# crowsonkb/style-transfer-pytorch

Hardware: AMD Instinct MI355X
Metric: optimizer iterations/sec (higher is better)
Workload: dtype f32 (3x3 convs: fp16x3 split-plane MFMA, fp32 accumulate); 1 GPU; 512x512 single-scale hot loop (closure + Adam + clamp + EMA), 1 style image 512x512, VGG-19 synthetic weights, max pooling; parallelism=single GPU

## Files before the change

include/st_amd.h:

```cpp
#ifndef ST_AMD_H
#define ST_AMD_H

#ifdef __cplusplus
extern "C" {
#endif

#define ST_AMD_ABI_VERSION 2

#define ST_NUM_CONVS 13
#define ST_NUM_STYLE_LAYERS 5
#define ST_CONTENT_LAYER 22
#define ST_NUM_LOSS_TERMS 7

enum st_pooling { ST_POOL_MAX = 0, ST_POOL_AVERAGE = 1, ST_POOL_L2 = 2 };

typedef struct st_net st_net;
typedef struct st_plan st_plan;

const char* st_last_error(void);
int st_abi_version(void);
const char* st_compiled_arch(void);
long long st_max_pixels(void);
int st_has_experiments(void);
int st_env_switches(const char** names, int capacity);
// ... 125 lines not shown
int st_fabric_selftest(st_fabric* fabric, void* stream, int timeout_ms);
int st_plan_closure_run(st_plan* plan, st_fabric* fabric, void* stream);
long long st_qn_strip_state_bytes(long long count, int world);
int st_qn_strip_dots(void* state, long long count, int rank, int world, const float* grad, st_exchange* gather,
                     void* stream);
int st_qn_strip_apply(void* state, long long count, int world, float* image, const float* grad, float* ema_value,
                      double ema_decay, void* stream);
int st_plan_qn_strip_step(st_plan* plan, st_fabric* fabric, float* image, float* grad, void* state, float* ema_value,
                          double ema_decay, void* stream);
int st_plan_losses(st_plan* plan, float** losses);
int st_plan_term_losses(st_plan* plan, float** terms, int* count);
int st_plan_forward_begin(st_plan* plan, const float* image, int last_layer);
int st_plan_moment_sums(st_plan* plan, int layer, float* sums, void* stream);

int st_plan_set_graph(st_plan* plan, int enable);

int st_plan_profile_enable(st_plan* plan, int enable);
int st_plan_profile_read(st_plan* plan, long long* launches, double* millis, double* flops);
int st_plan_profile_read_hbm(st_plan* plan, int category, long long* launches, double* millis, double* bytes);

int st_op_sqrtm_ns(const float* a, float* root, int n, void* stream);
int st_op_sqrtm_ns_backward(const float* root, const float* grad_root, float* grad_a, int n, void* stream);
int st_op_sqrtm_ns_backward_diag(const float* root, float grad_diag, float* grad_a, int n, void* stream);
int st_op_tv_loss(const float* image, int height, int width, float* loss_out, float* grad_out, void* stream);
int st_op_conv3x3(const float* in, const float* weight, const float* bias, float* out, int cin, int cout,
                  int height, int width, int relu, int precision, void* stream);
int st_op_conv3x3_dgrad(const float* grad_out, const float* relu_out, const float* weight, float* grad_in,
                        int cin, int cout, int height, int width, int precision, void* stream);
int st_op_conv3x3_strip(const float* in, const float* halo, int has_up, int has_down, const float* weight,
                        const float* bias, float* out, int cin, int cout, int height, int width, int relu, int dgrad,
                        int precision, void* stream);
int st_op_conv3x3_strip_ex(const float* in, const float* halo, int has_up, int has_down, const float* weight,
                           const float* bias, float* out, const float* out_mask, int cin, int cout, int height, int width,
                           int relu, int dgrad, int accumulate, int overlap, int precision, void* stream);

int st_op_conv1x1(const float* in, const float* weight, const float* bias, float* out, int cin, int cout,
                  long long npix, int precision, void* stream);

int st_op_pool2x2(const float* in, float* out, int channels, int height, int width, int mode, void* stream);
int st_op_pool2x2_backward(const float* in, const float* grad_out, float* grad_in, int channels, int height, int width,
                           int mode, void* stream);


typedef struct st_head st_head;
int st_head_create(st_head** out, int kind, int channels, int height, int width, int precision);
int st_head_destroy(st_head* head);
// ... 96 lines not shown
```

style-transfer-pytorch_amd/csrc/st_common.h:

```cpp
#pragma once

#include <hip/hip_runtime.h>

#include <algorithm>
#include <atomic>
#include <cstdarg>
#include <cstdio>
#include <string>

namespace st {

typedef float f32x16 __attribute__((ext_vector_type(16)));
typedef float f32x4 __attribute__((ext_vector_type(4)));
typedef float f32x2 __attribute__((ext_vector_type(2)));

constexpr int kWave = 64;

void set_error(const char* fmt, ...);
const char* get_error();

#define ST_HIP(expr)                                                                           \
    do {                                                                                       \
        hipError_t _e = (expr);                                                                \
        if (_e != hipSuccess) {                                                                \
// ... 106 lines not shown
    const float *mean, *mean_t, *cov, *cov_t, *root;
    int n;
    float weight;
    float* loss_out;
    float* gdiag_out;
};
__device__ __forceinline__ float w2_gdiag(const W2LossJob& j) { return -2.f * (j.weight / (float)j.n); }
__device__ __forceinline__ void w2_loss_block(const W2LossJob& j, float* scratch) {
#pragma clang fp contract(off)
    float sm = 0.f, sc = 0.f;
    for (int i = threadIdx.x; i < j.n; i += 256) {
        const float d = j.mean[i] - j.mean_t[i];
        sm += d * d;
        const size_t ii = (size_t)i * j.n + i;
        sc += (j.cov_t[ii] + j.cov[ii]) - 2.f * j.root[ii];
    }
    sm = block_sum_256(sm, scratch);
    sc = block_sum_256(sc, scratch);
    if (threadIdx.x == 0) {
        const float fn = (float)j.n;
        j.loss_out[0] = (sm / fn + sc / fn) * j.weight;
        j.gdiag_out[0] = w2_gdiag(j);
    }
}

static inline int ceil_div(int a, int b) { return (a + b - 1) / b; }

struct ConvProblem {
    const float* in;
    const float* mask;
    const float* wgt;
    const float* bias;
    float* out;
    int cin, cout, height, width;
    int taps;
    int relu;
    int accumulate;
    float* scratch;
    const float* in_halo;
    int has_up, has_down;
    int tune;
    const void* wgt_split;
    int planes;
    int elem;
    unsigned int* amax_word;
    int amax_measure;
// ... 129 lines not shown
int launch_pool_bwd(const float* in, const float* grad_out, float* grad_in, int channels, int height,
                    int width, int mode, hipStream_t s);

struct GramWorkspace {
    float* partial;
    float* partial_sum;
    int max_splits;
};
int gram_choose_splits(int channels, long long npix, int max_splits);
long long gram_per_split(long long npix, int splits);
bool gram_wide_tiles(int channels, long long npix);
int launch_gram_partial(const float* feat, int channels, long long npix, int splits, GramWorkspace ws,
                        hipStream_t s, const unsigned int* bound = nullptr, const float* sqrt_mask = nullptr);
int launch_gram_finalize(GramWorkspace ws, int channels, long long npix, int splits, float* mean, float* srm,
                         hipStream_t s, float* cov = nullptr, float cov_eps = 0.f,
                         float mask_sum = 0.f);

enum GemmEpilogue {
    EPI_SCALE = 0,
    EPI_IDENT_MINUS = 1,
    EPI_DIFF = 2,
    EPI_DEV_SQRT_SCALE = 3
};
struct GemmProblem {
    const float* a1; const float* b1;
    const float* a2; const float* b2; const float* b2sub;
    float* d;
    int ta1, tb1, ta2;
    int epilogue;
    float c, ci;
    const float* dev_scalar;
    int n;
    float* sumsq_partials;
};
bool gemm_sumsq_fusable(int n);
struct GemmBatch {
    GemmProblem p[6];
    int count;
    int n;
};
int launch_gemm_batch(const GemmBatch& b, hipStream_t s);
bool head_dgrad_small_applies(int channels, long long npix);
int launch_head_dgrad_small(const float* ssym, const float* feat, const float* bias, const float* mask, float* out, int channels,
                            long long npix, unsigned int* out_amax, hipStream_t s);

struct NSWorkspace {
    float *y0, *y1, *z0, *z1, *t;
    float *a0, *a1, *q0, *q1, *e, *atq, *qa;
    float* scalars;
    _Float16* planes;
    unsigned int* chain_sync;
    int chain_launches;
    float* chain_arena;
};
constexpr int kNsChainArenaMats = 132;

struct NsChainJob {
    int n;
    int tile0, tiles;
    int forward, backward;
    const float* m;
    const float* m_partials;
// ... 306 lines not shown
```

style-transfer-pytorch_amd/csrc/st_ops.hip:

```cpp
#include <cstdlib>
#include <vector>

#include "../../include/st_amd.h"
#include "st_common.h"

namespace st {
namespace {

struct OpScratch {
    hipStream_t stream;
    std::vector<void*> buffers;
    std::vector<hipEvent_t> events;
    explicit OpScratch(hipStream_t s) : stream(s) {}
    OpScratch(const OpScratch&) = delete;
    OpScratch& operator=(const OpScratch&) = delete;
    ~OpScratch() {
        hipStreamSynchronize(stream);
        for (void* b : buffers) hipFree(b);
        for (hipEvent_t e : events) hipEventDestroy(e);
    }
    template <class T>
    int alloc(T** out, size_t bytes) {
        void* p = nullptr;
        ST_HIP(hipMalloc(&p, bytes));
// ... 38 lines not shown
int st_op_sqrtm_ns_backward(const float* root, const float* grad_root, float* grad_a, int n, void* stream) {
    ST_REQUIRE(root && grad_root && grad_a, "st_op_sqrtm_ns_backward: null argument");
    hipStream_t s = static_cast<hipStream_t>(stream);
    OpScratch tmp(s);
    float* base = nullptr;
    if (tmp.alloc(&base, ns_workspace_floats(n) * sizeof(float))) return 1;
    NSWorkspace ws{};
    ns_workspace_carve(ws, base, n);
    return ns_workspace_reset(ws, s) || ns_sqrt_backward(root, grad_root, nullptr, grad_a, n, ws, s);
}

int st_op_sqrtm_ns_backward_diag(const float* root, float grad_diag, float* grad_a, int n, void* stream) {
    ST_REQUIRE(root && grad_a, "st_op_sqrtm_ns_backward_diag: null argument");
    hipStream_t s = static_cast<hipStream_t>(stream);
    OpScratch tmp(s);
    float *base = nullptr, *gd = nullptr;
    if (tmp.alloc(&base, ns_workspace_floats(n) * sizeof(float)) || tmp.alloc(&gd, 256)) return 1;
    ST_HIP(hipMemcpyAsync(gd, &grad_diag, sizeof(float), hipMemcpyHostToDevice, s));
    NSWorkspace ws{};
    ns_workspace_carve(ws, base, n);
    int rc = ns_workspace_reset(ws, s) || ns_sqrt_backward(root, nullptr, gd, grad_a, n, ws, s);
    hipStreamSynchronize(s);
    if (!rc) rc = ns_chain_check(ws, "st_op_sqrtm_ns_backward_diag");
    return rc;
}

int st_op_sqrtm_time(int n, int iters, double* fwd_us, double* bwd_us, void* stream) {
    ST_REQUIRE(fwd_us && bwd_us && iters > 0, "st_op_sqrtm_time: bad argument");
    hipStream_t s = static_cast<hipStream_t>(stream);
    const size_t nn = (size_t)n * n;
    OpScratch tmp(s);
    float *base = nullptr, *a = nullptr, *root = nullptr, *g = nullptr, *ga = nullptr, *gd = nullptr;
    if (tmp.alloc(&base, ns_workspace_floats(n) * 4) || tmp.alloc(&a, nn * 4) || tmp.alloc(&root, nn * 4) ||
        tmp.alloc(&g, nn * 4) || tmp.alloc(&ga, nn * 4) || tmp.alloc(&gd, 256))
        return 1;
    std::vector<float> h(nn, 0.f);
    unsigned x = 777u;
    for (size_t i = 0; i < nn; ++i) { x = x * 1664525u + 1013904223u; h[i] = ((int)(x >> 9) % 2001 - 1000) * 1e-4f; }
    for (int i = 0; i < n; ++i)
        for (int j = 0; j < i; ++j) h[(size_t)i * n + j] = h[(size_t)j * n + i];
    for (int i = 0; i < n; ++i) h[(size_t)i * n + i] = 1.0f + 0.1f * (i % 7);
    ST_HIP(hipMemcpy(a, h.data(), nn * 4, hipMemcpyHostToDevice));
    ST_HIP(hipMemcpy(g, h.data(), nn * 4, hipMemcpyHostToDevice));
    NSWorkspace ws{};
    ns_workspace_carve(ws, base, n);
    if (ns_workspace_reset(ws, s)) return 1;
// ... 267 lines not shown
```

style-transfer-pytorch_amd/csrc/st_smallgemm.hip:

```cpp
#include <cstdint>
#include <cstdlib>

#include "st_common.h"

namespace st {
namespace {

template <int KW>
struct Operand {
    float v[KW / 8][4];
};

template <int N, int KW>
__device__ __forceinline__ void load_operand(Operand<KW>& o, const float* __restrict__ base, bool rowk, int row0,
                                             int k0, int l31, int half) {
    if (rowk) {
        const float* src = base + (size_t)(row0 + l31) * N + k0 + 4 * half;
#pragma unroll
        for (int kb = 0; kb < KW / 8; ++kb) {
            const f32x4 t = *reinterpret_cast<const f32x4*>(src + kb * 8);
            o.v[kb][0] = t[0]; o.v[kb][1] = t[1]; o.v[kb][2] = t[2]; o.v[kb][3] = t[3];
        }
    } else {
        const float* src = base + (size_t)(k0 + 4 * half) * N + row0 + l31;
// ... 3 lines not shown
            for (int e = 0; e < 4; ++e) o.v[kb][e] = src[(size_t)(kb * 8 + e) * N];
    }
}

template <int N, int WV>
__device__ __forceinline__ void gemm_tile(const GemmProblem& pr, int tile, float (*red)[16][64]) {
    constexpr int KW = N / WV;
    constexpr int RPT = 16 / WV;
    const int tid = threadIdx.x, lane = tid & 63;
    const int wave = __builtin_amdgcn_readfirstlane(tid >> 6);
    const int l31 = lane & 31, half = lane >> 5;
    constexpr int nt = N / 32;
    const int m0 = (tile / nt) * 32, n0 = (tile % nt) * 32;
    const int k0 = wave * KW;
    const bool two = (pr.epilogue == EPI_DIFF);

    Operand<KW> a, b, a2, b2, bs;
    load_operand<N, KW>(a, pr.a1, !pr.ta1, m0, k0, l31, half);
    load_operand<N, KW>(b, pr.b1, pr.tb1 != 0, n0, k0, l31, half);
    if (two) {
        load_operand<N, KW>(a2, pr.a2, false, m0, k0, l31, half);
        load_operand<N, KW>(b2, pr.b2, false, n0, k0, l31, half);
        load_operand<N, KW>(bs, pr.b2sub, false, n0, k0, l31, half);
    }
    f32x16 acc1, acc2;
#pragma unroll
    for (int r = 0; r < 16; ++r) { acc1[r] = 0.f; acc2[r] = 0.f; }
#pragma unroll
    for (int kb = 0; kb < KW / 8; ++kb)
#pragma unroll
        for (int e = 0; e < 4; ++e) acc1 = __builtin_amdgcn_mfma_f32_32x32x2f32(a.v[kb][e], b.v[kb][e], acc1, 0, 0, 0);
    if (two) {
#pragma unroll
        for (int kb = 0; kb < KW / 8; ++kb)
#pragma unroll
            for (int e = 0; e < 4; ++e)
                acc2 = __builtin_amdgcn_mfma_f32_32x32x2f32(a2.v[kb][e], b2.v[kb][e] - bs.v[kb][e], acc2, 0, 0, 0);
    }

    auto reduce = [&](const f32x16& acc, float (&out)[RPT]) __attribute__((always_inline)) {
#pragma unroll
        for (int r = 0; r < 16; ++r) red[wave][r][lane] = acc[r];
        __syncthreads();
#pragma unroll
        for (int rr = 0; rr < RPT; ++rr) {
            float part[WV];
// ... 17 lines not shown
    if (pr.epilogue == EPI_DEV_SQRT_SCALE) dscale = sqrtf(pr.dev_scalar[0]);
#pragma unroll
    for (int rr = 0; rr < RPT; ++rr) {
        const int r = wave * RPT + rr;
        const int orow = m0 + (r & 3) + 8 * (r >> 2) + 4 * half;
        const int ocol = n0 + l31;
        float v;
        if (pr.epilogue == EPI_SCALE) {
            v = s1[rr] * pr.c;
        } else if (pr.epilogue == EPI_IDENT_MINUS) {
            v = ((orow == ocol ? pr.ci : 0.f) - s1[rr]) * pr.c;
        } else if (pr.epilogue == EPI_DIFF) {
            v = (s1[rr] - s2[rr]) * pr.c;
        } else {
            v = s1[rr] * dscale;
        }
        pr.d[(size_t)orow * N + ocol] = v;
    }
}

template <int N, int WV>
__global__ __launch_bounds__(WV * 64) void gemm_batch_kernel(GemmBatch batch) {
    __shared__ float red[WV][16][64];
    gemm_tile<N, WV>(batch.p[blockIdx.y], blockIdx.x, red);
}

__global__ __launch_bounds__(512) void gemm_mixed_kernel(GemmBatch batch) {
    __shared__ float red[8][16][64];
    const GemmProblem& pr = batch.p[blockIdx.y];
    const int n = pr.n ? pr.n : batch.n;
    const int tiles = (n / 32) * (n / 32);
    if ((int)blockIdx.x >= tiles) return;
    if (n == 64) gemm_tile<64, 8>(pr, blockIdx.x, red);
    else if (n == 128) gemm_tile<128, 8>(pr, blockIdx.x, red);
    else gemm_tile<256, 8>(pr, blockIdx.x, red);
}

constexpr int kPitch = 36;
constexpr int kImage = 32 * kPitch;

template <int RK>
struct TileRegs {
    f32x4 v[RK / 8];
};

template <int N, int RK>
__device__ __forceinline__ void load_slice(TileRegs<RK>& t, const float* __restrict__ base, bool rowk,
                                           int row0, int k0, int lane) {
    if (rowk) {
        constexpr int C4 = RK / 4;
#pragma unroll
// ... 210 lines not shown
        const int orow = m0 + (r & 3) + 8 * (r >> 2) + 4 * half;
        const size_t at = (size_t)orow * npix + n0 + l31;
        float v = part[0] + bias[orow];
        if (mask != nullptr) v = (mask[at] > 0.f) ? v : 0.f;
        out[at] = v;
        amax = max(amax, abs_bits(v));
    }
    if (out_amax) amax_commit(amax, out_amax);
}

GemmProblem plain(const float* a, const float* b, float* d, float c = 1.f, int ta = 0, int tb = 0) {
    GemmProblem p{};
    p.a1 = a; p.b1 = b; p.d = d; p.ta1 = ta; p.tb1 = tb; p.epilogue = EPI_SCALE; p.c = c;
    return p;
}

}

int launch_gemm_batch(const GemmBatch& b, hipStream_t s) {
    ST_REQUIRE(b.count >= 1 && b.count <= 6, "gemm: batch count out of range");
    for (int i = 0; i < b.count; ++i) {
        ST_REQUIRE(!(b.p[i].ta1 && b.p[i].tb1), "gemm: A^T @ B^T is not implemented");
        ST_REQUIRE(b.p[i].epilogue != EPI_DIFF || (b.p[i].ta2 == 1), "gemm: second product must be A2^T @ (B2 - B2sub)");
    }
    bool mixed = false;
    int nmax = 0;
    for (int i = 0; i < b.count; ++i) {
        const int ni = b.p[i].n ? b.p[i].n : b.n;
        mixed = mixed || ni != b.n;
        nmax = std::max(nmax, ni);
        ST_REQUIRE(!b.p[i].n || ni == 64 || ni == 128 || ni == 256, "gemm: a problem's own size must be 64, 128 or 256");
    }
    if (mixed) {
        ST_REQUIRE(b.n <= 256, "gemm: mixed batches are for n <= 256");
        for (int i = 0; i < b.count; ++i) ST_REQUIRE(b.p[i].epilogue != EPI_DIFF, "gemm: mixed batches have single products");
        hipLaunchKernelGGL(gemm_mixed_kernel, dim3((nmax / 32) * (nmax / 32), b.count), dim3(512), 0, s, b);
        ST_LAUNCH_CHECK();
        return 0;
    }
    for (int i = 0; i < b.count; ++i)
        ST_REQUIRE(!b.p[i].sumsq_partials || (!mixed && gemm_sumsq_fusable(b.n)), "gemm: fused sums of squares exist for n = 512 only");
    const int nt = b.n / 32;
    const dim3 grid(nt * nt, b.count);
    switch (b.n) {
        case 64: hipLaunchKernelGGL((gemm_batch_kernel<64, 2>), grid, dim3(128), 0, s, b); break;
        case 128: hipLaunchKernelGGL((gemm_batch_kernel<128, 4>), grid, dim3(256), 0, s, b); break;
        case 256: hipLaunchKernelGGL((gemm_batch_kernel<256, 8>), grid, dim3(512), 0, s, b); break;
        case 512: hipLaunchKernelGGL((gemm_staged_kernel<512, 4>), grid, dim3(256), 0, s, b); break;
        default: ST_REQUIRE(false, "gemm: n must be 64, 128, 256 or 512 (got %d)", b.n);
    }
    ST_LAUNCH_CHECK();
    return 0;
}

bool gemm_sumsq_fusable(int n) {
    static Option on("ST_NS_FUSED_SUMSQ", 1);
    return on.get() != 0 && n == 512;
}

bool head_dgrad_small_applies(int channels, long long npix) {
    static Option on("ST_HEAD_SMALL_GEMM", 1);
    return on.get() != 0 && (channels == 64 || channels == 128 || channels == 256 || channels == 512) && npix >= 32 &&
           npix <= 1024 && npix % 32 == 0;
}

int launch_head_dgrad_small(const float* ssym, const float* feat, const float* bias, const float* mask, float* out, int channels,
                            long long npix, unsigned int* out_amax, hipStream_t s) {
    ST_REQUIRE(head_dgrad_small_applies(channels, npix), "head gradient (small tap): unsupported shape %d x %lld", channels, npix);
    ST_REQUIRE((reinterpret_cast<uintptr_t>(ssym) & 15) == 0, "head gradient (small tap): Ssym must be 16-byte aligned");
    const dim3 grid(channels / 32, (unsigned)(npix / 32));
    switch (channels) {
// ... 76 lines not shown

int ns_sqrt_chain(const float* const* m, float* const* root, float* const* grad_m, const int* n, NSWorkspace* const* ws,
                  const int* m_partials, const W2LossJob* loss, int lanes, hipStream_t s) {
    ST_REQUIRE(lanes >= 1 && lanes <= 3, "ns chain: 1 to 3 heads per launch");
    NsChainLaunch launch{};
    launch.count = lanes;
    for (int l = 0; l < lanes; ++l) {
        NsChainJob& j = launch.job[l];
        j = ns_chain_job(*ws[l], n[l]);
        j.forward = 1; j.backward = 1;
        j.m = m[l]; j.root = root[l]; j.grad_m = grad_m[l];
        if (m_partials && m_partials[l] > 0) { j.m_partials = ws[l]->scalars + 8; j.m_nparts = m_partials[l]; }
        ST_REQUIRE(loss && loss[l].loss_out, "ns chain: the combined form carries the head's W2 scalars");
        j.loss = loss[l];
    }
    return launch_ns_chain(launch, s);
}

static bool ns_skip_identity() {
    static Option opt("ST_NS_SKIP_IDENTITY", 1);
    return opt.get() != 0;
}

int ns_sqrt_forward(const float* m, float* root, int n, NSWorkspace& ws, hipStream_t s, int m_partials, int* root_partials) {
    if (root_partials) *root_partials = 0;
    if (ns_f16_forward() && ns_f16_applies(n) && ws.planes) return ns_sqrt_forward_f16(m, root, n, ws, s);
    if ((ns_chain_mask() & 8) && ws.chain_sync) {
        NsChainLaunch launch{};
        launch.count = 1;
        NsChainJob& j = launch.job[0];
        j = ns_chain_job(ws, n);
        j.forward = 1;
        j.m = m; j.root = root;
        if (m_partials > 0) { j.m_partials = ws.scalars + 8; j.m_nparts = m_partials; }
        return launch_ns_chain(launch, s);
    }
    const bool shortcut = ns_skip_identity();
    if (launch_ns_prepare(m, n, ws.scalars + 0, ws.scalars + 8, ws.y0, nullptr, nullptr, shortcut ? ws.z1 : ws.z0, s, shortcut,
                          nullptr, m_partials))
        return 1;
    float *y = ws.y0, *yn = ws.y1, *z = ws.z0, *zn = ws.z1;
    if (shortcut) {
        GemmBatch b{};
        b.n = n; b.count = 1;
        b.p[0] = plain(y, zn, yn);
        if (launch_gemm_batch(b, s)) return 1;
        std::swap(y, yn);
        std::swap(z, zn);
    }
    for (int it = shortcut ? 1 : 0; it < 12; ++it) {
        const bool last = (it == 11);
        GemmBatch b1{};
        b1.n = n; b1.count = 1;
        b1.p[0] = plain(z, y, ws.t);
        b1.p[0].epilogue = EPI_IDENT_MINUS; b1.p[0].ci = 3.f; b1.p[0].c = 0.5f;
        if (launch_gemm_batch(b1, s)) return 1;
        GemmBatch b2{};
        b2.n = n;
        if (!last) {
            b2.count = 2;
            b2.p[0] = plain(y, ws.t, yn);
            b2.p[1] = plain(ws.t, z, zn);
        } else {
            b2.count = 1;
            b2.p[0] = plain(y, ws.t, root);
            b2.p[0].epilogue = EPI_DEV_SQRT_SCALE; b2.p[0].dev_scalar = ws.scalars + 0;
            if (root_partials && gemm_sumsq_fusable(n)) {
                b2.p[0].sumsq_partials = ws.scalars + 8;
// ... 3 lines not shown
        if (launch_gemm_batch(b2, s)) return 1;
        float* tmp = y; y = yn; yn = tmp;
        tmp = z; z = zn; zn = tmp;
    }
    return 0;
}

namespace {
GemmProblem sized(GemmProblem p, int n) {
    p.n = n;
    return p;
}
int batch_n(const int* n, int lanes) {
    int m = 0;
    for (int l = 0; l < lanes; ++l) m = std::max(m, n[l]);
    return m;
}
}

int ns_sqrt_forward_lockstep(const float* const* m, float* const* root, const int* n, NSWorkspace* const* wsp, int lanes,
                             hipStream_t s) {
    ST_REQUIRE(lanes >= 1 && lanes <= 3, "ns forward (lockstep): 1 to 3 chains");
    const bool shortcut = ns_skip_identity();
    float *y[3], *yn[3], *z[3], *zn[3];
    for (int l = 0; l < lanes; ++l) {
        ST_REQUIRE(n[l] == 64 || n[l] == 128 || n[l] == 256, "ns forward (lockstep): n must be 64, 128 or 256");
        NSWorkspace& ws = *wsp[l];
        if (launch_ns_prepare(m[l], n[l], ws.scalars + 0, ws.scalars + 8, ws.y0, nullptr, nullptr, shortcut ? ws.z1 : ws.z0, s,
                              shortcut))
            return 1;
        y[l] = ws.y0; yn[l] = ws.y1; z[l] = ws.z0; zn[l] = ws.z1;
    }
    const int nb = batch_n(n, lanes);
    if (shortcut) {
        GemmBatch b{};
        b.n = nb; b.count = lanes;
        for (int l = 0; l < lanes; ++l) b.p[l] = sized(plain(y[l], zn[l], yn[l]), n[l]);
        if (launch_gemm_batch(b, s)) return 1;
        for (int l = 0; l < lanes; ++l) {
            std::swap(y[l], yn[l]);
            std::swap(z[l], zn[l]);
        }
    }
    for (int it = shortcut ? 1 : 0; it < 12; ++it) {
        const bool last = (it == 11);
        GemmBatch b1{};
        b1.n = nb; b1.count = lanes;
        for (int l = 0; l < lanes; ++l) {
            b1.p[l] = sized(plain(z[l], y[l], wsp[l]->t), n[l]);
            b1.p[l].epilogue = EPI_IDENT_MINUS; b1.p[l].ci = 3.f; b1.p[l].c = 0.5f;
        }
        if (launch_gemm_batch(b1, s)) return 1;
        GemmBatch b2{};
        b2.n = nb;
        for (int l = 0; l < lanes; ++l) {
            if (!last) {
                b2.p[b2.count++] = sized(plain(y[l], wsp[l]->t, yn[l]), n[l]);
                b2.p[b2.count++] = sized(plain(wsp[l]->t, z[l], zn[l]), n[l]);
            } else {
                GemmProblem pr = sized(plain(y[l], wsp[l]->t, root[l]), n[l]);
                pr.epilogue = EPI_DEV_SQRT_SCALE; pr.dev_scalar = wsp[l]->scalars + 0;
                b2.p[b2.count++] = pr;
            }
        }
        if (launch_gemm_batch(b2, s)) return 1;
        for (int l = 0; l < lanes; ++l) {
            std::swap(y[l], yn[l]);
            std::swap(z[l], zn[l]);
        }
    }
    return 0;
}

int ns_sqrt_backward_diag_lockstep(const float* const* root, const float* const* grad_diag, float* const* grad_m, const int* n,
                                   NSWorkspace* const* wsp, int lanes, hipStream_t s, const W2LossJob* loss) {
    ST_REQUIRE(lanes >= 1 && lanes <= 3, "ns backward (lockstep): 1 to 3 chains");
    float *a[3], *an[3], *q[3], *qn[3];
    for (int l = 0; l < lanes; ++l) {
        NSWorkspace& ws = *wsp[l];
        if (launch_ns_prepare(root[l], n[l], ws.scalars + 1, ws.scalars + 8, ws.a0, nullptr, grad_diag[l], ws.q0, s, false,
                              loss ? &loss[l] : nullptr))
            return 1;
        a[l] = ws.a0; an[l] = ws.a1; q[l] = ws.q0; qn[l] = ws.q1;
    }
    const int nb = batch_n(n, lanes);
    for (int it = 0; it < 12; ++it) {
        const bool last = (it == 11);
        GemmBatch b1{};
        b1.n = nb; b1.count = lanes;
        for (int l = 0; l < lanes; ++l) {
            b1.p[l] = sized(plain(a[l], a[l], wsp[l]->e), n[l]);
            b1.p[l].epilogue = EPI_IDENT_MINUS; b1.p[l].ci = 3.f; b1.p[l].c = 1.f;
        }
        if (launch_gemm_batch(b1, s)) return 1;
        GemmBatch b2{};
        b2.n = nb;
        for (int l = 0; l < lanes; ++l) {
            b2.p[b2.count++] = sized(plain(q[l], wsp[l]->e, last ? grad_m[l] : qn[l], last ? 0.25f : 0.5f), n[l]);
            if (!last) b2.p[b2.count++] = sized(plain(a[l], wsp[l]->e, an[l], 0.5f), n[l]);
        }
        if (launch_gemm_batch(b2, s)) return 1;
        for (int l = 0; l < lanes; ++l) {
            std::swap(a[l], an[l]);
            std::swap(q[l], qn[l]);
        }
    }
    return 0;
}

int ns_sqrt_backward(const float* root, const float* grad_root, const float* grad_diag, float* grad_m, int n,
                     NSWorkspace& ws, hipStream_t s, const W2LossJob* loss, int root_partials) {
    ST_REQUIRE(!loss || (grad_diag && loss->gdiag_out == grad_diag), "ns backward: a W2 job defines the diagonal seed it rides with");
    {
        if (grad_diag && !ns_full_backward() && (ns_chain_mask() & 8) && ws.chain_sync) {
            NsChainLaunch launch{};
            launch.count = 1;
            NsChainJob& j = launch.job[0];
            j = ns_chain_job(ws, n);
            j.backward = 1;
            j.root = const_cast<float*>(root); j.grad_m = grad_m;
            j.gdiag_dev = grad_diag;
            if (loss) j.loss = *loss;
            return launch_ns_chain(launch, s);
        }
        if (grad_diag && !ns_full_backward() && ns_f16_applies(n) && ws.planes)
            return ns_sqrt_backward_diag_f16(root, grad_diag, grad_m, n, ws, s, loss, root_partials);
    }
    if (launch_ns_prepare(root, n, ws.scalars + 1, ws.scalars + 8, ws.a0, grad_diag ? nullptr : grad_root, grad_diag,
                          ws.q0, s, false, loss, root_partials))
        return 1;
    float *a = ws.a0, *an = ws.a1, *q = ws.q0, *qn = ws.q1;
    const bool reduced = grad_diag != nullptr && !ns_full_backward();
    for (int it = 0; it < 12; ++it) {
        const bool last = (it == 11);
        GemmBatch b1{};
        b1.n = n; b1.count = reduced ? 1 : 3;
        b1.p[0] = plain(a, a, ws.e);
        b1.p[0].epilogue = EPI_IDENT_MINUS; b1.p[0].ci = 3.f; b1.p[0].c = 1.f;
        if (!reduced) {
            b1.p[1] = plain(a, q, ws.atq, 1.f, 1);
            b1.p[2] = plain(q, a, ws.qa);
        }
        if (launch_gemm_batch(b1, s)) return 1;
        GemmBatch b2{};
        b2.n = n; b2.count = last ? 1 : 2;
        GemmProblem& pq = b2.p[0];
        pq = plain(q, ws.e, last ? grad_m : qn, last ? 0.25f : 0.5f);
        if (!reduced) {
            pq.epilogue = EPI_DIFF;
            pq.a2 = a; pq.ta2 = 1; pq.b2 = ws.atq; pq.b2sub = ws.qa;
        }
        if (!last) b2.p[1] = plain(a, ws.e, an, 0.5f);
        if (launch_gemm_batch(b2, s)) return 1;
        float* tmp = a; a = an; an = tmp;
        tmp = q; q = qn; qn = tmp;
    }
    return 0;
}

}
```

style-transfer-pytorch_amd/style_transfer/_hip.py:

```python

import ctypes
import os

import torch

_PKG_ROOT = os.path.dirname(os.path.dirname(os.path.abspath(__file__)))
_LIB_CANDIDATES = (os.path.join(_PKG_ROOT, 'lib', 'libst_amd.so'),
                   os.path.join(os.path.dirname(os.path.abspath(__file__)), 'lib', 'libst_amd.so'))
LIB_PATH = next((c for c in _LIB_CANDIDATES if os.path.exists(c)), _LIB_CANDIDATES[0])

_c_float_p = ctypes.c_void_p
TAPS = (1, 3, 4, 6, 8, 9, 11, 13, 15, 17, 18, 20, 22, 24, 26, 27, 29)
DEFAULT_CONTENT_LAYERS, DEFAULT_STYLE_LAYERS = (22,), (1, 6, 11, 20, 29)
CONTENT_LOSSES, STYLE_LOSSES = ('mse', 'scaled_mse'), ('w2', 'gram')
NEAREST_METRICS = ('l2', 'cosine', 'centered_cosine')
_lib = None


class HipLibraryError(RuntimeError):
    pass


class Exchange(ctypes.Structure):
    _fields_ = [('kind', ctypes.c_int), ('count', ctypes.c_longlong), ('send_up', ctypes.c_void_p),
# ... 86 lines not shown
        'st_qn_strip_apply': (i32, [vp, i64, i32, vp, vp, vp, f64, vp]),
        'st_plan_qn_strip_step': (i32, [vp, vp, vp, vp, vp, vp, f64, vp]),
        'st_plan_create_strip': (i32, [pp, vp, i32, i32, i32, i32]),
        'st_plan_closure_begin': (i32, [vp, vp, vp]),
        'st_plan_set_rank': (i32, [vp, i32, i32]),
        'st_plan_closure_next': (i32, [vp, ctypes.POINTER(Exchange), vp]),
        'st_fabric_unique_id': (i32, [ctypes.c_char_p]),
        'st_fabric_create': (i32, [pp, ctypes.c_char_p, ctypes.c_char_p, i32, i32, i32]),
        'st_fabric_destroy': (i32, [vp]),
        'st_fabric_abort': (i32, [vp]),
        'st_fabric_selftest': (i32, [vp, vp, i32]),
        'st_plan_closure_run': (i32, [vp, vp, vp]),
        'st_plan_losses': (i32, [vp, pp]),
        'st_plan_debug_read': (i32, [vp, i32, ctypes.POINTER(f32), i32]),
        'st_plan_forward_begin': (i32, [vp, vp, i32]),
        'st_plan_moment_sums': (i32, [vp, i32, vp, vp]),
        'st_plan_set_graph': (i32, [vp, i32]),
        'st_plan_profile_enable': (i32, [vp, i32]),
        'st_plan_profile_read': (i32, [vp, ctypes.POINTER(i64), ctypes.POINTER(f64), ctypes.POINTER(f64)]),
        'st_plan_profile_read_hbm': (i32, [vp, i32, ctypes.POINTER(i64), ctypes.POINTER(f64), ctypes.POINTER(f64)]),
        'st_op_sqrtm_ns': (i32, [vp, vp, i32, vp]),
        'st_op_sqrtm_ns_backward': (i32, [vp, vp, vp, i32, vp]),
        'st_op_sqrtm_ns_backward_diag': (i32, [vp, f32, vp, i32, vp]),
        'st_op_tv_loss': (i32, [vp, i32, i32, vp, vp, vp]),
        'st_op_sqrtm_time': (i32, [i32, i32, ctypes.POINTER(f64), ctypes.POINTER(f64), vp]),
        'st_op_mfma_rate': (i32, [i32, i32, i32, i32, ctypes.POINTER(f64), ctypes.POINTER(f64), vp]),
        'st_op_mfma_valu_rate': (i32, [i32, i32, i32, i32, i32, i32, i32, ctypes.POINTER(f64), ctypes.POINTER(f64),
                                       ctypes.POINTER(f64), vp]),
        'st_op_grid_barrier_time': (i32, [i32, i32, i32, i32, ctypes.POINTER(f64), ip, vp]),
        'st_op_winograd_consumer_rate': (i32, [i32, i32, ctypes.POINTER(f64), vp]),
        'st_op_conv3x3_time': (i32, [i32, i32, i32, i32, i32, i32, i32, ctypes.POINTER(f64), vp]),
        'st_op_conv3x3': (i32, [vp, vp, vp, vp, i32, i32, i32, i32, i32, i32, vp]),
        'st_op_conv3x3_dgrad': (i32, [vp, vp, vp, vp, i32, i32, i32, i32, i32, vp]),
        'st_op_conv3x3_strip': (i32, [vp, vp, i32, i32, vp, vp, vp, i32, i32, i32, i32, i32, i32, i32, vp]),
        'st_op_conv3x3_strip_ex': (i32, [vp, vp, i32, i32, vp, vp, vp, vp, i32, i32, i32, i32, i32, i32, i32, i32, i32, vp]),
        'st_op_conv1x1': (i32, [vp, vp, vp, vp, i32, i32, i64, i32, vp]),
        'st_op_pool2x2': (i32, [vp, vp, i32, i32, i32, i32, vp]),
        'st_op_pool2x2_backward': (i32, [vp, vp, vp, i32, i32, i32, i32, vp]),
        'st_head_create': (i32, [pp, i32, i32, i32, i32, i32]),
        'st_head_destroy': (i32, [vp]),
        'st_head_device_bytes': (i64, [vp]),
        'st_head_state_floats': (i64, [vp]),
        'st_head_moments': (i32, [vp, vp, vp, vp, vp]),
        'st_op_gram_split_plan': (i32, [i32, i64, i32, ip, ctypes.POINTER(i64), ip]),
        'st_head_forward': (i32, [vp, vp, vp, vp, vp, vp, f32, vp, vp, vp]),
        'st_head_backward': (i32, [vp, vp, vp, vp, vp, vp]),
# ... 926 lines not shown
        _check(lib.st_op_sqrtm_ns(_ptr(a.contiguous()), _ptr(root), n, _stream()))
    return root


def op_sqrtm_ns_backward(root, grad_root):
    lib = load_library()
    n = root.shape[-1]
    ga = torch.empty(root.shape, dtype=root.dtype, device=root.device)
    with torch.cuda.device(root.device):
        _check(lib.st_op_sqrtm_ns_backward(_ptr(root.contiguous()), _ptr(grad_root.contiguous()), _ptr(ga), n,
                                           _stream()))
    return ga


def op_sqrtm_ns_backward_diag(root, grad_diag):
    lib = load_library()
    n = root.shape[-1]
    ga = torch.empty(root.shape, dtype=root.dtype, device=root.device)
    with torch.cuda.device(root.device):
        _check(lib.st_op_sqrtm_ns_backward_diag(_ptr(root.contiguous()), float(grad_diag), _ptr(ga), n, _stream()))
    return ga


def op_sqrtm_time(n, iters=20):
    lib = load_library()
    f, b = ctypes.c_double(), ctypes.c_double()
    _check(lib.st_op_sqrtm_time(int(n), int(iters), ctypes.byref(f), ctypes.byref(b), _stream()))
    return f.value, b.value


def op_mfma_rate(lds_reads=0, waves=8, steps=20000, launches=10):
    lib = load_library()
    t, m = ctypes.c_double(), ctypes.c_double()
    _check(lib.st_op_mfma_rate(int(lds_reads), int(waves), int(steps), int(launches), ctypes.byref(t),
                               ctypes.byref(m), _stream()))
    return t.value, m.value


def op_mfma_valu_rate(lds_reads, waves, steps, valu_waves, valu_steps, valu_prio=0, launches=10):
    lib = load_library()
    t, m = ctypes.c_double(), ctypes.c_double()
    c = (ctypes.c_double * 2)()
    _check(lib.st_op_mfma_valu_rate(int(lds_reads), int(waves), int(steps), int(launches), int(valu_waves),
                                    int(valu_steps), int(valu_prio), ctypes.byref(t), ctypes.byref(m), c, _stream()))
    return t.value, m.value, c[0], c[1]

# ... 487 lines not shown
```

Measured before the change: 450.2 it/s.

## Fold Newton-Schulz prepare step into first GEMM and ride W2 loss

Adds operand-transform modes to the small GEMM batch so that the first Newton-Schulz product normalises its inputs by the Frobenius norm. The norm is reduced from sum-of-squares partials inside the kernel, and the identity-based initial operands are built on load. This removes the separate prepare launch that materialised the normalised matrices. The W2 loss reduction is also folded into an extra block of the first backward GEMM launch. A lockstep test entry point is exposed as well. The change adds per-tile norm reductions that each block recomputes and more branching in operand loading, and it applies only for n <= 256.

Result: no change. 448.0 it/s (-0.5%).

```diff
diff --git a/include/st_amd.h b/include/st_amd.h
--- a/include/st_amd.h
+++ b/include/st_amd.h
@@ -171,6 +171,8 @@
 int st_op_sqrtm_ns(const float* a, float* root, int n, void* stream);
 int st_op_sqrtm_ns_backward(const float* root, const float* grad_root, float* grad_a, int n, void* stream);
 int st_op_sqrtm_ns_backward_diag(const float* root, float grad_diag, float* grad_a, int n, void* stream);
+int st_op_sqrtm_ns_lockstep(const float* const* a, float* const* root, float* const* grad_a, const int* n, int lanes,
+                            float grad_diag, void* stream);
 int st_op_tv_loss(const float* image, int height, int width, float* loss_out, float* grad_out, void* stream);
 int st_op_conv3x3(const float* in, const float* weight, const float* bias, float* out, int cin, int cout,
                   int height, int width, int relu, int precision, void* stream);
diff --git a/style-transfer-pytorch_amd/csrc/st_common.h b/style-transfer-pytorch_amd/csrc/st_common.h
--- a/style-transfer-pytorch_amd/csrc/st_common.h
+++ b/style-transfer-pytorch_amd/csrc/st_common.h
@@ -152,6 +152,12 @@
         j.loss_out[0] = (sm / fn + sc / fn) * j.weight;
         j.gdiag_out[0] = w2_gdiag(j);
     }
+}
+
+__device__ __forceinline__ void w2_loss_rider(const W2LossJob& j, float* scratch) {
+    if (threadIdx.x < 4) scratch[threadIdx.x] = 0.f;
+    __syncthreads();
+    w2_loss_block(j, scratch);
 }
 
 static inline int ceil_div(int a, int b) { return (a + b - 1) / b; }
@@ -327,6 +333,43 @@
     EPI_DIFF = 2,
     EPI_DEV_SQRT_SCALE = 3
 };
+enum GemmOperandMode {
+    OPER_PLAIN = 0,
+    OPER_DIV = 1,
+    OPER_T0 = 2,
+    OPER_DIAG = 3
+};
+struct GemmOpen {
+    int amode, bmode;
+    const float* partials; int nparts;
+    const float* norm;
+    float* norm_out;
+    float* t0_out;
+    const float* gdiag;
+};
+__device__ __forceinline__ float open_norm(const GemmOpen& o) {
+    if (o.partials == nullptr) return o.norm[0];
+    const int lane = threadIdx.x & 63;
+    float w[4];
+#pragma unroll
+    for (int v = 0; v < 4; ++v) {
+        float s = 0.f;
+        for (int i = 64 * v + lane; i < o.nparts; i += 256) s += o.partials[i];
+#pragma unroll
+        for (int off = 32; off > 0; off >>= 1) s += __shfl_xor(s, off, 64);
+        w[v] = s;
+    }
+    return sqrtf((w[0] + w[1]) + (w[2] + w[3]));
+}
+__device__ __forceinline__ float open_value(int mode, float x, float d, float dv, bool diag) {
+#pragma clang fp contract(off)
+    if (mode == OPER_DIV) return x / d;
+    if (mode == OPER_T0) return ((diag ? 3.f : 0.f) - x / d) * 0.5f;
+    if (mode == OPER_DIAG) return diag ? dv : 0.f;
+    return x;
+}
+bool ns_fold_open();
+
 struct GemmProblem {
     const float* a1; const float* b1;
     const float* a2; const float* b2; const float* b2sub;
@@ -337,12 +380,15 @@
     const float* dev_scalar;
     int n;
     float* sumsq_partials;
+    GemmOpen open;
 };
 bool gemm_sumsq_fusable(int n);
 struct GemmBatch {
     GemmProblem p[6];
     int count;
     int n;
+    W2LossJob loss[3];
+    int loss_count;
 };
 int launch_gemm_batch(const GemmBatch& b, hipStream_t s);
 bool head_dgrad_small_applies(int channels, long long npix);
diff --git a/style-transfer-pytorch_amd/csrc/st_ops.hip b/style-transfer-pytorch_amd/csrc/st_ops.hip
--- a/style-transfer-pytorch_amd/csrc/st_ops.hip
+++ b/style-transfer-pytorch_amd/csrc/st_ops.hip
@@ -84,6 +84,31 @@
     int rc = ns_workspace_reset(ws, s) || ns_sqrt_backward(root, nullptr, gd, grad_a, n, ws, s);
     hipStreamSynchronize(s);
     if (!rc) rc = ns_chain_check(ws, "st_op_sqrtm_ns_backward_diag");
+    return rc;
+}
+
+int st_op_sqrtm_ns_lockstep(const float* const* a, float* const* root, float* const* grad_a, const int* n, int lanes,
+                            float grad_diag, void* stream) {
+    ST_REQUIRE(a && root && grad_a && n && lanes >= 1 && lanes <= 3, "st_op_sqrtm_ns_lockstep: 1 to 3 chains");
+    hipStream_t s = static_cast<hipStream_t>(stream);
+    OpScratch tmp(s);
+    NSWorkspace ws[3]{};
+    NSWorkspace* wsp[3] = {};
+    const float *croot[3] = {}, *gds[3] = {};
+    float* gd = nullptr;
+    if (tmp.alloc(&gd, 256)) return 1;
+    ST_HIP(hipMemcpyAsync(gd, &grad_diag, sizeof(float), hipMemcpyHostToDevice, s));
+    for (int l = 0; l < lanes; ++l) {
+        ST_REQUIRE(a[l] && root[l] && grad_a[l] && (n[l] == 64 || n[l] == 128 || n[l] == 256), "st_op_sqrtm_ns_lockstep: n must be 64, 128 or 256");
+        float* base = nullptr;
+        if (tmp.alloc(&base, ns_workspace_floats(n[l]) * sizeof(float))) return 1;
+        ns_workspace_carve(ws[l], base, n[l]);
+        if (ns_workspace_reset(ws[l], s)) return 1;
+        wsp[l] = &ws[l]; croot[l] = root[l]; gds[l] = gd;
+    }
+    int rc = ns_sqrt_forward_lockstep(a, root, n, wsp, lanes, s) ||
+             ns_sqrt_backward_diag_lockstep(croot, gds, grad_a, n, wsp, lanes, s);
+    hipStreamSynchronize(s);
     return rc;
 }
 
diff --git a/style-transfer-pytorch_amd/csrc/st_smallgemm.hip b/style-transfer-pytorch_amd/csrc/st_smallgemm.hip
--- a/style-transfer-pytorch_amd/csrc/st_smallgemm.hip
+++ b/style-transfer-pytorch_amd/csrc/st_smallgemm.hip
@@ -49,6 +49,20 @@
         load_operand<N, KW>(a2, pr.a2, false, m0, k0, l31, half);
         load_operand<N, KW>(b2, pr.b2, false, n0, k0, l31, half);
         load_operand<N, KW>(bs, pr.b2sub, false, n0, k0, l31, half);
+    }
+    if (pr.open.amode | pr.open.bmode) {
+        const float d = open_norm(pr.open);
+        const float dv = pr.open.amode == OPER_DIAG ? pr.open.gdiag[0] / d : 0.f;
+#pragma unroll
+        for (int kb = 0; kb < KW / 8; ++kb)
+#pragma unroll
+            for (int e = 0; e < 4; ++e) {
+                const int k = k0 + 4 * half + 8 * kb + e;
+                a.v[kb][e] = open_value(pr.open.amode, a.v[kb][e], d, dv, k == m0 + l31);
+                b.v[kb][e] = open_value(pr.open.bmode, b.v[kb][e], d, dv, k == n0 + l31);
+                if (pr.open.bmode == OPER_T0 && k >= m0 && k < m0 + 32) pr.open.t0_out[(size_t)k * N + n0 + l31] = b.v[kb][e];
+            }
+        if (pr.open.norm_out && tile == 0 && tid == 0) pr.open.norm_out[0] = d;
     }
     f32x16 acc1, acc2;
 #pragma unroll
@@ -112,11 +126,19 @@
 template <int N, int WV>
 __global__ __launch_bounds__(WV * 64) void gemm_batch_kernel(GemmBatch batch) {
     __shared__ float red[WV][16][64];
+    if (batch.loss_count && blockIdx.x == gridDim.x - 1) {
+        if ((int)blockIdx.y < batch.loss_count) w2_loss_rider(batch.loss[blockIdx.y], &red[0][0][0]);
+        return;
+    }
     gemm_tile<N, WV>(batch.p[blockIdx.y], blockIdx.x, red);
 }
 
 __global__ __launch_bounds__(512) void gemm_mixed_kernel(GemmBatch batch) {
     __shared__ float red[8][16][64];
+    if (batch.loss_count && blockIdx.x == gridDim.x - 1) {
+        if ((int)blockIdx.y < batch.loss_count) w2_loss_rider(batch.loss[blockIdx.y], &red[0][0][0]);
+        return;
+    }
     const GemmProblem& pr = batch.p[blockIdx.y];
     const int n = pr.n ? pr.n : batch.n;
     const int tiles = (n / 32) * (n / 32);
@@ -373,7 +395,19 @@
     for (int i = 0; i < b.count; ++i) {
         ST_REQUIRE(!(b.p[i].ta1 && b.p[i].tb1), "gemm: A^T @ B^T is not implemented");
         ST_REQUIRE(b.p[i].epilogue != EPI_DIFF || (b.p[i].ta2 == 1), "gemm: second product must be A2^T @ (B2 - B2sub)");
-    }
+        const GemmOpen& o = b.p[i].open;
+        if (o.amode | o.bmode) {
+            ST_REQUIRE(b.p[i].epilogue != EPI_DIFF && (o.partials ? o.nparts > 0 : o.norm != nullptr), "gemm: an opening product is single and has a norm");
+            ST_REQUIRE(o.amode != OPER_T0 && o.bmode != OPER_DIAG && (o.amode != OPER_DIAG || o.gdiag), "gemm: opening operand modes");
+            ST_REQUIRE(o.bmode != OPER_T0 || (o.t0_out && !b.p[i].tb1), "gemm: the first step's t is an untransposed B operand");
+        }
+    }
+    ST_REQUIRE(b.loss_count >= 0 && b.loss_count <= 3 && b.loss_count <= b.count, "gemm: at most one W2 job per problem");
+    for (int i = 0; i < b.loss_count; ++i)
+        ST_REQUIRE(b.loss[i].loss_out && b.loss[i].n == (b.p[i].n ? b.p[i].n : b.n), "gemm: W2 job %d rides with problem %d of its size", i, i);
+    const unsigned riders = b.loss_count > 0 ? 1 : 0;
+    bool opens = false;
+    for (int i = 0; i < b.count; ++i) opens = opens || (b.p[i].open.amode | b.p[i].open.bmode) != 0;
     bool mixed = false;
     int nmax = 0;
     for (int i = 0; i < b.count; ++i) {
@@ -385,19 +419,22 @@
     if (mixed) {
         ST_REQUIRE(b.n <= 256, "gemm: mixed batches are for n <= 256");
         for (int i = 0; i < b.count; ++i) ST_REQUIRE(b.p[i].epilogue != EPI_DIFF, "gemm: mixed batches have single products");
-        hipLaunchKernelGGL(gemm_mixed_kernel, dim3((nmax / 32) * (nmax / 32), b.count), dim3(512), 0, s, b);
+        hipLaunchKernelGGL(gemm_mixed_kernel, dim3((nmax / 32) * (nmax / 32) + riders, b.count), dim3(512), 0, s, b);
         ST_LAUNCH_CHECK();
         return 0;
     }
     for (int i = 0; i < b.count; ++i)
         ST_REQUIRE(!b.p[i].sumsq_partials || (!mixed && gemm_sumsq_fusable(b.n)), "gemm: fused sums of squares exist for n = 512 only");
     const int nt = b.n / 32;
-    const dim3 grid(nt * nt, b.count);
+    const dim3 grid(nt * nt + riders, b.count);
     switch (b.n) {
         case 64: hipLaunchKernelGGL((gemm_batch_kernel<64, 2>), grid, dim3(128), 0, s, b); break;
         case 128: hipLaunchKernelGGL((gemm_batch_kernel<128, 4>), grid, dim3(256), 0, s, b); break;
         case 256: hipLaunchKernelGGL((gemm_batch_kernel<256, 8>), grid, dim3(512), 0, s, b); break;
-        case 512: hipLaunchKernelGGL((gemm_staged_kernel<512, 4>), grid, dim3(256), 0, s, b); break;
+        case 512:
+            ST_REQUIRE(!opens && !riders, "gemm: opening products and W2 riders exist for n <= 256 only");
+            hipLaunchKernelGGL((gemm_staged_kernel<512, 4>), grid, dim3(256), 0, s, b);
+            break;
         default: ST_REQUIRE(false, "gemm: n must be 64, 128, 256 or 512 (got %d)", b.n);
     }
     ST_LAUNCH_CHECK();
@@ -520,6 +557,40 @@
     return opt.get() != 0;
 }
 
+bool ns_fold_open() {
+    static Option opt("ST_NS_FOLD_OPEN", 1);
+    return opt.get() != 0;
+}
+
+namespace {
+GemmProblem forward_opening(const float* m, float* y1, float* t0, NSWorkspace& ws, int parts) {
+    GemmProblem p = plain(m, m, y1);
+    p.open.amode = OPER_DIV; p.open.bmode = OPER_T0;
+    p.open.partials = ws.scalars + 8; p.open.nparts = parts;
+    p.open.norm_out = ws.scalars + 0;
+    p.open.t0_out = t0;
+    return p;
+}
+GemmProblem backward_opening_e(const float* root, NSWorkspace& ws, int parts) {
+    GemmProblem p = plain(root, root, ws.e);
+    p.epilogue = EPI_IDENT_MINUS; p.ci = 3.f; p.c = 1.f;
+    p.open.amode = OPER_DIV; p.open.bmode = OPER_DIV;
+    p.open.partials = ws.scalars + 8; p.open.nparts = parts;
+    p.open.norm_out = ws.scalars + 1;
+    return p;
+}
+GemmProblem backward_opening_q(const float* root, const float* gdiag, float* q1, NSWorkspace& ws) {
+    GemmProblem p = plain(root, ws.e, q1, 0.5f);
+    p.open.amode = OPER_DIAG; p.open.gdiag = gdiag; p.open.norm = ws.scalars + 1;
+    return p;
+}
+GemmProblem backward_opening_a(const float* root, float* a1, NSWorkspace& ws) {
+    GemmProblem p = plain(root, ws.e, a1, 0.5f);
+    p.open.amode = OPER_DIV; p.open.norm = ws.scalars + 1;
+    return p;
+}
+}
+
 int ns_sqrt_forward(const float* m, float* root, int n, NSWorkspace& ws, hipStream_t s, int m_partials, int* root_partials) {
     if (root_partials) *root_partials = 0;
     if (ns_f16_forward() && ns_f16_applies(n) && ws.planes) return ns_sqrt_forward_f16(m, root, n, ws, s);
@@ -534,14 +605,18 @@
         return launch_ns_chain(launch, s);
     }
     const bool shortcut = ns_skip_identity();
-    if (launch_ns_prepare(m, n, ws.scalars + 0, ws.scalars + 8, ws.y0, nullptr, nullptr, shortcut ? ws.z1 : ws.z0, s, shortcut,
-                          nullptr, m_partials))
+    const bool fold = shortcut && ns_fold_open() && n <= 256;
+    if (fold) {
+        if (m_partials <= 0 && launch_sumsq_partials(m, (long long)n * n, ws.scalars + 8, &m_partials, s)) return 1;
+    } else if (launch_ns_prepare(m, n, ws.scalars + 0, ws.scalars + 8, ws.y0, nullptr, nullptr, shortcut ? ws.z1 : ws.z0, s,
+                                 shortcut, nullptr, m_partials)) {
         return 1;
+    }
     float *y = ws.y0, *yn = ws.y1, *z = ws.z0, *zn = ws.z1;
     if (shortcut) {
         GemmBatch b{};
         b.n = n; b.count = 1;
-        b.p[0] = plain(y, zn, yn);
+        b.p[0] = fold ? forward_opening(m, yn, zn, ws, m_partials) : plain(y, zn, yn);
         if (launch_gemm_batch(b, s)) return 1;
         std::swap(y, yn);
         std::swap(z, zn);
@@ -591,20 +666,26 @@
                              hipStream_t s) {
     ST_REQUIRE(lanes >= 1 && lanes <= 3, "ns forward (lockstep): 1 to 3 chains");
     const bool shortcut = ns_skip_identity();
+    const bool fold = shortcut && ns_fold_open();
+    int parts[3] = {};
     float *y[3], *yn[3], *z[3], *zn[3];
     for (int l = 0; l < lanes; ++l) {
         ST_REQUIRE(n[l] == 64 || n[l] == 128 || n[l] == 256, "ns forward (lockstep): n must be 64, 128 or 256");
         NSWorkspace& ws = *wsp[l];
-        if (launch_ns_prepare(m[l], n[l], ws.scalars + 0, ws.scalars + 8, ws.y0, nullptr, nullptr, shortcut ? ws.z1 : ws.z0, s,
-                              shortcut))
+        if (fold) {
+            if (launch_sumsq_partials(m[l], (long long)n[l] * n[l], ws.scalars + 8, &parts[l], s)) return 1;
+        } else if (launch_ns_prepare(m[l], n[l], ws.scalars + 0, ws.scalars + 8, ws.y0, nullptr, nullptr, shortcut ? ws.z1 : ws.z0,
+                                     s, shortcut)) {
             return 1;
+        }
         y[l] = ws.y0; yn[l] = ws.y1; z[l] = ws.z0; zn[l] = ws.z1;
     }
     const int nb = batch_n(n, lanes);
     if (shortcut) {
         GemmBatch b{};
         b.n = nb; b.count = lanes;
-        for (int l = 0; l < lanes; ++l) b.p[l] = sized(plain(y[l], zn[l], yn[l]), n[l]);
+        for (int l = 0; l < lanes; ++l)
+            b.p[l] = sized(fold ? forward_opening(m[l], yn[l], zn[l], *wsp[l], parts[l]) : plain(y[l], zn[l], yn[l]), n[l]);
         if (launch_gemm_batch(b, s)) return 1;
         for (int l = 0; l < lanes; ++l) {
             std::swap(y[l], yn[l]);
@@ -645,11 +726,16 @@
                                    NSWorkspace* const* wsp, int lanes, hipStream_t s, const W2LossJob* loss) {
     ST_REQUIRE(lanes >= 1 && lanes <= 3, "ns backward (lockstep): 1 to 3 chains");
     float *a[3], *an[3], *q[3], *qn[3];
+    const bool fold = ns_fold_open();
+    int parts[3] = {};
     for (int l = 0; l < lanes; ++l) {
         NSWorkspace& ws = *wsp[l];
-        if (launch_ns_prepare(root[l], n[l], ws.scalars + 1, ws.scalars + 8, ws.a0, nullptr, grad_diag[l], ws.q0, s, false,
-                              loss ? &loss[l] : nullptr))
+        if (fold) {
+            if (launch_sumsq_partials(root[l], (long long)n[l] * n[l], ws.scalars + 8, &parts[l], s)) return 1;
+        } else if (launch_ns_prepare(root[l], n[l], ws.scalars + 1, ws.scalars + 8, ws.a0, nullptr, grad_diag[l], ws.q0, s, false,
+                                     loss ? &loss[l] : nullptr)) {
             return 1;
+        }
         a[l] = ws.a0; an[l] = ws.a1; q[l] = ws.q0; qn[l] = ws.q1;
     }
     const int nb = batch_n(n, lanes);
@@ -657,14 +743,23 @@
         const bool last = (it == 11);
         GemmBatch b1{};
         b1.n = nb; b1.count = lanes;
+        const bool opening = fold && it == 0;
         for (int l = 0; l < lanes; ++l) {
             b1.p[l] = sized(plain(a[l], a[l], wsp[l]->e), n[l]);
             b1.p[l].epilogue = EPI_IDENT_MINUS; b1.p[l].ci = 3.f; b1.p[l].c = 1.f;
+            if (opening) {
+                b1.p[l] = sized(backward_opening_e(root[l], *wsp[l], parts[l]), n[l]);
+                if (loss) b1.loss[b1.loss_count++] = loss[l];
+            }
         }
         if (launch_gemm_batch(b1, s)) return 1;
         GemmBatch b2{};
         b2.n = nb;
-        for (int l = 0; l < lanes; ++l) {
+        for (int l = 0; l < lanes && opening; ++l) {
+            b2.p[b2.count++] = sized(backward_opening_q(root[l], grad_diag[l], qn[l], *wsp[l]), n[l]);
+            b2.p[b2.count++] = sized(backward_opening_a(root[l], an[l], *wsp[l]), n[l]);
+        }
+        for (int l = 0; l < lanes && !opening; ++l) {
             b2.p[b2.count++] = sized(plain(q[l], wsp[l]->e, last ? grad_m[l] : qn[l], last ? 0.25f : 0.5f), n[l]);
             if (!last) b2.p[b2.count++] = sized(plain(a[l], wsp[l]->e, an[l], 0.5f), n[l]);
         }
@@ -695,9 +790,14 @@
         if (grad_diag && !ns_full_backward() && ns_f16_applies(n) && ws.planes)
             return ns_sqrt_backward_diag_f16(root, grad_diag, grad_m, n, ws, s, loss, root_partials);
     }
-    if (launch_ns_prepare(root, n, ws.scalars + 1, ws.scalars + 8, ws.a0, grad_diag ? nullptr : grad_root, grad_diag,
-                          ws.q0, s, false, loss, root_partials))
+    const bool reduced_form = grad_diag != nullptr && !ns_full_backward();
+    const bool fold = reduced_form && ns_fold_open() && n <= 256;
+    if (fold) {
+        if (root_partials <= 0 && launch_sumsq_partials(root, (long long)n * n, ws.scalars + 8, &root_partials, s)) return 1;
+    } else if (launch_ns_prepare(root, n, ws.scalars + 1, ws.scalars + 8, ws.a0, grad_diag ? nullptr : grad_root, grad_diag,
+                                 ws.q0, s, false, loss, root_partials)) {
         return 1;
+    }
     float *a = ws.a0, *an = ws.a1, *q = ws.q0, *qn = ws.q1;
     const bool reduced = grad_diag != nullptr && !ns_full_backward();
     for (int it = 0; it < 12; ++it) {
@@ -710,6 +810,11 @@
             b1.p[1] = plain(a, q, ws.atq, 1.f, 1);
             b1.p[2] = plain(q, a, ws.qa);
         }
+        const bool opening = fold && it == 0;
+        if (opening) {
+            b1.p[0] = backward_opening_e(root, ws, root_partials);
+            if (loss) { b1.loss[0] = *loss; b1.loss_count = 1; }
+        }
         if (launch_gemm_batch(b1, s)) return 1;
         GemmBatch b2{};
         b2.n = n; b2.count = last ? 1 : 2;
@@ -720,6 +825,10 @@
             pq.a2 = a; pq.ta2 = 1; pq.b2 = ws.atq; pq.b2sub = ws.qa;
         }
         if (!last) b2.p[1] = plain(a, ws.e, an, 0.5f);
+        if (opening) {
+            b2.p[0] = backward_opening_q(root, grad_diag, qn, ws);
+            b2.p[1] = backward_opening_a(root, an, ws);
+        }
         if (launch_gemm_batch(b2, s)) return 1;
         float* tmp = a; a = an; an = tmp;
         tmp = q; q = qn; qn = tmp;
diff --git a/style-transfer-pytorch_amd/style_transfer/_hip.py b/style-transfer-pytorch_amd/style_transfer/_hip.py
--- a/style-transfer-pytorch_amd/style_transfer/_hip.py
+++ b/style-transfer-pytorch_amd/style_transfer/_hip.py
@@ -132,6 +132,7 @@
         'st_op_sqrtm_ns': (i32, [vp, vp, i32, vp]),
         'st_op_sqrtm_ns_backward': (i32, [vp, vp, vp, i32, vp]),
         'st_op_sqrtm_ns_backward_diag': (i32, [vp, f32, vp, i32, vp]),
+        'st_op_sqrtm_ns_lockstep': (i32, [ctypes.POINTER(vp), ctypes.POINTER(vp), ctypes.POINTER(vp), ctypes.POINTER(i32), i32, f32, vp]),
         'st_op_tv_loss': (i32, [vp, i32, i32, vp, vp, vp]),
         'st_op_sqrtm_time': (i32, [i32, i32, ctypes.POINTER(f64), ctypes.POINTER(f64), vp]),
         'st_op_mfma_rate': (i32, [i32, i32, i32, i32, ctypes.POINTER(f64), ctypes.POINTER(f64), vp]),
@@ -1104,6 +1105,19 @@
     return ga
 
 
+def op_sqrtm_ns_lockstep(mats, grad_diag):
+    lib = load_library()
+    mats = [m.contiguous() for m in mats]
+    roots = [torch.empty_like(m) for m in mats]
+    grads = [torch.empty_like(m) for m in mats]
+    k = len(mats)
+    pa, pr, pg = ((ctypes.c_void_p * k)(*[_ptr(t).value for t in ts]) for ts in (mats, roots, grads))
+    ns = (ctypes.c_int * k)(*[m.shape[-1] for m in mats])
+    with torch.cuda.device(mats[0].device):
+        _check(lib.st_op_sqrtm_ns_lockstep(pa, pr, pg, ns, k, float(grad_diag), _stream()))
+    return roots, grads
+
+
 def op_sqrtm_time(n, iters=20):
     lib = load_library()
     f, b = ctypes.c_double(), ctypes.c_double()
```
